# empymod/emg3d

Measured on AMD Instinct MI355X. Metric: Mcells/s per multigrid cycle, higher is better.
Workload: dtype c128

## Files before the change

emg3d_amd/csrc/emg3d_hip.hip:

```cpp
#include "../../include/emg3d_hip.h"

#include <cstring>
#include <new>

#include <chrono>
#include "mg.hpp"
#include "receivers.hpp"
#include "source.hpp"
#include "gradient.hpp"
#include "regrid.hpp"

#define EMG3D_HIP_VERSION EMG3D_HIP_ABI_VERSION

namespace {

template <class T>
MG<T>* as(emg3d_mg_t* mg) { return static_cast<MG<T>*>(reinterpret_cast<emg3d_mg*>(mg)); }

static int current_device() { int d = 0; if (hipGetDevice(&d) != hipSuccess) { (void)hipGetLastError(); d = 0; } return d; }

template <class T> static T scalar_of(double re, double im);
template <> double scalar_of<double>(double re, double) { return re; }
template <> c128 scalar_of<c128>(double re, double im) { return mk(re, im); }

// ... 460 lines not shown
    HIP_TRY(hipMemcpy(dv, values, (size_t)tot * sizeof(T), hipMemcpyHostToDevice));
    int rc = interp3d_device<T>(nullptr, dv, nn, 0, 1, nx, nx * ny, pts, n, xi, method, has_fill != 0, fill, cval, nullptr, scr, dout);
    if (rc == 0 && hipMemcpy(out, dout, (size_t)n * sizeof(T), hipMemcpyDeviceToHost) != hipSuccess) rc = (int)hipGetLastError();
        return rc;
}

}

template <class T>
static void* efield_ptr(MG<T>* m) {
    if (hipSetDevice(m->device) != hipSuccess) { (void)hipGetLastError(); return nullptr; }
    T* p = m->sel_e();
    m->check_launch();
    return m->err ? nullptr : (void*)p;
}

template <class T>
static int sweep_plan_impl(i64 nx, i64 ny, i64 nz, int dir, int order, int nsys, int cu_count, char* name, int64_t* info) {
    SweepKnobs K;
    if (cu_count > 0) K.simds = 4 * (i64)cu_count;
    else sweep_device_knobs<T>(K, current_device());
    K.order = order; K.nsys = nsys;
    const SweepPlan p = plan_sweep(K, SweepShape{{nx, ny, nz}, (int)sizeof(T)}, dir - 1);
    memcpy(name, p.name, sizeof p.name);
    info[0] = p.nmax; info[1] = p.lpw; info[2] = p.rounds; info[3] = p.fac_kind; info[4] = p.split ? 1 : 0; info[5] = p.big ? 1 : 0;
    return 0;
}

template <class T>
static int fuse_plan_impl(i64 nx, i64 ny, i64 nz, int dir, int order, int nsys, int cu_count, int npass, int own, int max_seg, i64 budget, int64_t* info,
                          int64_t* ranges, i64 nranges) {
    SweepKnobs K;
    if (cu_count > 0) K.simds = 4 * (i64)cu_count;
    else sweep_device_knobs<T>(K, current_device());
    K.order = order; K.nsys = nsys;
    if (own > 0) K.fuse_own = own;
    if (max_seg > 0) K.fuse_max_seg = max_seg;
    if (budget > 0) K.fuse_max_bytes = budget;
    const SweepShape G{{nx, ny, nz}, (int)sizeof(T)};
    const FusePlan f = plan_fuse(K, G, dir - 1, npass);
    int P, Q;
    sweep_axes(dir - 1, P, Q);
    info[0] = f.fused ? 1 : 0; info[1] = f.axis ? Q : P; info[2] = f.g.nX; info[3] = f.g.own; info[4] = f.g.nslabs; info[5] = f.g.npass;
    info[6] = f.nw; info[7] = f.scratch_bytes;
    if (!f.fused || !ranges) return 0;
    const i64 per = 4 + 2 * (i64)npass;
    if (nranges < per * f.g.nslabs) return -2;
    for (int k = 0; k < f.g.nslabs; ++k) {
        int64_t* r = ranges + per * k;
        r[0] = fuse_x0(f.g, k); r[1] = fuse_x1(f.g, k);
        i64 a = -1, b = -1;
        for (int j = 0; j <= f.g.nX; ++j) if (fuse_owner(f.g, j) == k) { if (a < 0) a = j; b = j + 1; }
        r[2] = a; r[3] = b;
        for (int p = 0; p < npass; ++p) { r[4 + 2 * p] = fuse_lo(f.g, k, p); r[5 + 2 * p] = fuse_hi(f.g, k, p); }
    }
    return 0;
}

template <class T>
static int jvec_stage(MG<T>* m, const double* const hv[3], const double* dv[3]) {
    Level<T>& L = *m->lv0;
    double* stage = reinterpret_cast<double*>(L.r);
    const i64 n = L.nCells;
    int used = 0;
    for (int c = 0; c < 3; ++c) {
        dv[c] = nullptr;
        if (!hv[c]) continue;
        for (int q = 0; q < c; ++q) if (hv[q] == hv[c]) dv[c] = dv[q];
        if (dv[c]) continue;
        double* d = stage + (i64)used++ * n;
        HIP_TRY(hipMemcpyAsync(d, hv[c], (size_t)n * sizeof(double), hipMemcpyHostToDevice, m->stream));
        dv[c] = d;
    }
    return 0;
}

template <class T>
static int jvec_source_impl(MG<T>* m, int efield_vec, double smu0_re, double smu0_im, const double* vx, const double* vy,
                            const double* vz) {
    if (sizeof(T) == 8 && smu0_im != 0.0) return -2;
    HIP_TRY(hipSetDevice(m->device));
    Level<T>& L = *m->lv0;
    const T* fwd = m->vec(efield_vec);
    if (!fwd || efield_vec < 0) return -2;
    const double* hv[3] = {vx, vy, vz};
    const double* dv[3];
    { const int st = jvec_stage<T>(m, hv, dv); if (st) return st; }
    T* s = m->sel_s();
    if (m->broken) return (int)hipErrorOutOfMemory;
    hipLaunchKernelGGL(k_jvec_source<T>, dim3((unsigned)((L.nE + 255) / 256)), dim3(256), 0, m->stream, L.nC[0], L.nC[1], L.nC[2],
                       L.fl, fwd, smu0_re, smu0_im, dv[0], dv[1], dv[2], (const double*)L.h[0], (const double*)L.h[1],
                       (const double*)L.h[2], s, L.nE);
    m->source_changed();
    m->lv0->s_dense = true;
    m->check_launch();
    return finish(m);
}

template <class T>
static int jvec_source_b_impl(MG<T>* m, int fwd_bvec, double smu0_re, double smu0_im, const double* vx, const double* vy,
                              const double* vz, const int32_t* use) {
    if (sizeof(T) == 8 && smu0_im != 0.0) return -2;
    HIP_TRY(hipSetDevice(m->device));
    Level<T>& L = *m->lv0;
    if (fwd_bvec < 0 || fwd_bvec >= (int)m->bvecs.size()) return -2;
    const T* fwd = m->bvecs[(size_t)fwd_bvec];
// ... 1146 lines not shown
```

emg3d_amd/csrc/mg.hpp:

```cpp
#pragma once
#include <algorithm>
#include <cmath>
#include <cstdlib>
#include <cstring>
#include <map>
#include <memory>
#include <mutex>
#include <chrono>
#include <vector>

#include "common.hpp"
#include "smooth.hpp"
#include "stencil.hpp"
#include "gradient.hpp"
#include "regrid.hpp"
#include "smooth_qpl.hpp"
#include "smooth_qc.hpp"
#include "smooth_thm.hpp"
#include "smooth_tha.hpp"
#include "sweep_launch.hpp"
#include "sweep_plan.hpp"

template <class T>
struct Level {
    i64 nC[3];
    i64 nE, nCells;
    FieldLayout fl;
    CellLayout cl;
    std::vector<double> h_host[3], nodes[3], centers[3];
    double* h[3] = {nullptr, nullptr, nullptr};
    double* ih[3] = {nullptr, nullptr, nullptr};
    T* eta[3] = {nullptr, nullptr, nullptr};
    double* zeta = nullptr;
    unsigned char* sflag[3] = {nullptr, nullptr, nullptr};
    bool sflag_valid[3] = {false, false, false};
    bool s_dense = false;
    bool zeta_sep = false;
    T *s = nullptr, *e = nullptr, *r = nullptr;
    T *eT = nullptr, *sT = nullptr;
    T* etaT[3] = {nullptr, nullptr, nullptr};
    double* zetaT = nullptr;
    bool sT_valid = false;
    FieldLayout flT;
    CellLayout clT;
    T *eW[2] = {nullptr, nullptr}, *sW[2] = {nullptr, nullptr};
    double* zetaW[2] = {nullptr, nullptr};
    bool sW_valid[2] = {false, false};
    int e_home = 0;
    T* fac[3] = {nullptr, nullptr, nullptr};
    void* qd[3][4] = {{nullptr, nullptr, nullptr, nullptr}, {nullptr, nullptr, nullptr, nullptr}, {nullptr, nullptr, nullptr, nullptr}};
    unsigned qdn[3][4] = {{0, 0, 0, 0}, {0, 0, 0, 0}, {0, 0, 0, 0}};
    T* fz[3] = {nullptr, nullptr, nullptr};
    i64 fz_n[3] = {0, 0, 0};
    FusePlan fuse[3];
    int fuse_key[3] = {-1, -1, -1};
    std::vector<int> passes[3];
    i64 fac_lines[3] = {0, 0, 0};
    i64 fac_mid[3] = {0, 0, 0};
    int fac_kind[3] = {0, 0, 0};
    SweepPlan plan[3];
    int plan_key[3] = {-1, -1, -1};
};

struct Transfer {
    int sc = -1;
    int co[3] = {0, 0, 0};
    double* w[3][3] = {{nullptr, nullptr, nullptr}, {nullptr, nullptr, nullptr}, {nullptr, nullptr, nullptr}};
    int* pidx[3] = {nullptr, nullptr, nullptr};
    double* pwt[3] = {nullptr, nullptr, nullptr};
};

template <class T>
struct Hierarchy {
    std::vector<std::shared_ptr<Level<T>>> lv;
    std::vector<Transfer> tr;
};

class DevicePool {
    std::mutex mu;
    struct Parked { void* p; int tag; };
    std::multimap<std::pair<int, size_t>, Parked> free_blocks;
    size_t held = 0, cap;
public:
    DevicePool() {
        const char* g = getenv("EMG3D_POOL_GB");
        cap = (size_t)((g ? atof(g) : 96.0) * (double)((size_t)1 << 30));
    }
    void* take(int device, size_t nb, int tag = 0, bool* hit = nullptr) {
        std::lock_guard<std::mutex> lk(mu);
        if (hit) *hit = false;
        auto rng = free_blocks.equal_range({device, nb});
        if (rng.first == rng.second) return nullptr;
        auto pick = rng.second;
        for (auto it = rng.first; it != rng.second; ++it) if (it->second.tag == tag) { pick = it; break; }
        if (pick == rng.second && tag != 0)
            for (auto it = rng.first; it != rng.second; ++it) if (it->second.tag == 0) { pick = it; break; }
        if (pick == rng.second) pick = rng.first;
        if (hit) *hit = tag != 0 && pick->second.tag == tag;
        void* p = pick->second.p;
        free_blocks.erase(pick);
        held -= nb;
        return p;
    }
    bool give(int device, void* p, size_t nb, int tag = 0) {
        std::lock_guard<std::mutex> lk(mu);
        if (held + nb > cap) return false;
// ... 1005 lines not shown
        L.e_home = 0;
    }
    void e_to_w1(Level<T>& L) {
        if (L.e_home == 1) return;
        ensure_work(L, 1);
        convert_field(L, L.eW[1], L.e, 1, true, true);
        L.e_home = 1;
    }

    int lex_loop = (int)LAB_ENV("EMG3D_LEX_LOOP", 1);
    void line_args(Level<T>& L, int dir, LineArgs<T>& a, bool sweep) {
        if (dir == 0) { a.L = 0; a.P = 1; a.Q = 2; }
        else if (dir == 1) { a.L = 1; a.P = 0; a.Q = 2; }
        else { a.L = 2; a.P = 0; a.Q = 1; }
        const SweepPlan& P = plan(L, dir);
        const bool sp = sweep && P.split;
        const bool t = (sp && dir == 0) ? true : P.xt;
        const int w = (dir == 0) ? 0 : 1;
        for (int q = 0; q < 3; ++q) {
            a.nC[q] = L.nC[q]; a.eta[q] = t ? L.etaT[q] : L.eta[q]; a.h[q] = L.h[q]; a.ih[q] = L.ih[q];
        }
        a.fl = t ? L.flT : L.fl; a.cl = t ? L.clT : L.cl;
        a.split = sp ? 1 : 0;
        if (sp) { a.e = L.eW[w]; a.s = L.sW[w]; a.zeta = L.zetaW[w]; }
        else { a.e = t ? L.eT : L.e; a.s = t ? L.sT : L.s; a.zeta = t ? L.zetaT : L.zeta; }
        const i64 nP = L.nC[a.P], nQ = L.nC[a.Q];
        a.nA[0] = (nP - 0) / 2; a.nA[1] = (nP - 1) / 2;
        const i64 nB[2] = {(nQ - 0) / 2, (nQ - 1) / 2};
        a.nB2[0] = nB[0]; a.nB2[1] = nB[1];
        i64 o = 0;
        for (int c = 0; c < 4; ++c) { a.base[c] = o; o += a.nA[c & 1] * nB[c >> 1]; }
        a.nLinesTot = o;
        a.fac = L.fac[dir];
        a.mid = L.fac[dir] ? L.fac_mid[dir] : L.nC[a.L] - 1;
        a.qm = (L.fac[dir] && L.fac_kind[dir] == 3) ? 2 : 0;
        a.fcomp = (L.fac[dir] && L.fac_kind[dir] == 4) ? 1 : 0;
        a.zsep = (sweep && L.zeta_sep && use_zsep) ? 1 : 0;
        a.sflag = (sweep && sflag_on(L, dir) && L.sflag[dir] && L.sflag_valid[dir]) ? L.sflag[dir] : nullptr;
        a.xcd = xcd_map;
        a.tile = q_tile;
        {
            const int ax[3] = {a.L, a.P, a.Q};
            a.rs.ihL = a.ih[a.L]; a.rs.ihP = a.ih[a.P]; a.rs.ihQ = a.ih[a.Q];
            a.rs.hL = a.h[a.L]; a.rs.hP = a.h[a.P]; a.rs.hQ = a.h[a.Q];
            a.rs.nL = (unsigned)a.nC[a.L]; a.rs.slot0 = 0;
            a.rs.nP = (unsigned)a.nC[a.P]; a.rs.nQ = (unsigned)a.nC[a.Q];
            a.rs.csL = (unsigned)a.cl.st[a.L]; a.rs.csP = (unsigned)a.cl.st[a.P]; a.rs.csQ = (unsigned)a.cl.st[a.Q];
            for (int c = 0; c < 3; ++c) {
                a.rs.off[c] = (unsigned)a.fl.off[ax[c]];
                for (int d = 0; d < 3; ++d) a.rs.st[c][d] = (unsigned)a.fl.st[ax[c]][ax[d]];
            }
        }
        a.qd = nullptr; a.qdn = 0;
        a.fe = nullptr; a.fnE = 0; a.fax = a.fnX = a.fown = a.fns = a.fnp = 0; a.fseq = 0;
        for (int c = 0; c < 4; ++c) { a.fqd[c] = nullptr; a.fqdn[c] = 0; }
        a.qpl = P.NW; a.qM = P.M; a.seg = P.seg; a.qlpw = 0;
        a.tha = P.helpers;
        a.mode = 0; a.cP = a.cQ = 0; a.cntA = a.cntB = 0; a.t = a.jQ0 = a.cnt = 0;
        a.bt = sweep ? batch(L) : Batch();
    }

    void ensure_factor(Level<T>& L, int dir) {
        const SweepPlan& P = plan(L, dir);
        if (P.xt) ensure_transposed_model(L);
        if (L.fac[dir]) return;
        L.fac_lines[dir] = (L.nC[dir == 0 ? 1 : 0] - 1) * (L.nC[dir == 2 ? 1 : 2] - 1);
        L.fac[dir] = dalloc<T>(L.fac_lines[dir] * P.fac_entries);
        L.fac_mid[dir] = P.mid;
        L.fac_kind[dir] = P.fac_kind;
        if (P.fac_kind == 3) thm_attrs();
        compute_factor(L, dir);
    }
    void compute_factor(Level<T>& L, int dir) {
        LineArgs<T> a;
        line_args(L, dir, a, false);
        a.fac = L.fac[dir];
        a.fcomp = L.fac_kind[dir] == 4;
        if (L.fac_kind[dir] == 3) {
            a.mid = L.fac_mid[dir];
            const i64 nQ_ = L.nC[a.Q];
            const i64 nmax_ = a.nA[0] * ((nQ_ - 0) / 2);
            a.mode = 3;
            if (nmax_ > 0)
                MG_LAUNCH(k_line_factor_m<T>, dim3((unsigned)((nmax_ + EMG_LINE_BLOCK - 1) / EMG_LINE_BLOCK), 4),
                                   dim3(EMG_LINE_BLOCK), 0, stream, a);
            check_launch();
            return;
        }
        a.mid = L.fac_mid[dir];
        const i64 nQ = L.nC[a.Q];
        const i64 nB[2] = {(nQ - 0) / 2, (nQ - 1) / 2};
        a.mode = 3; a.cP = a.cQ = 0; a.cntA = a.cntB = 0;
        const i64 nmax = a.nA[0] * nB[0];
#ifdef EMG3D_LAB
        if (LAB_ENV("EMG3D_FACTOR_PER_COLOUR", 0)) {
            for (int c = 0; c < 4; ++c) {
                a.mode = 0; a.cP = c & 1; a.cQ = c >> 1; a.cntA = a.nA[a.cP]; a.cntB = nB[a.cQ];
                const i64 n = a.cntA * a.cntB;
                if (n > 0)
                    MG_LAUNCH(k_line_factor<T>, dim3((unsigned)((n + EMG_LINE_BLOCK - 1) / EMG_LINE_BLOCK)),
                                       dim3(EMG_LINE_BLOCK), 0, stream, a);
            }
            check_launch();
            return;
        }
#endif
        if (nmax > 0)
// ... 207 lines not shown
            L.eW[w] = cands[best];
            block_tag[cands[best]] = 1 + w;
            for (int k = 0; k < R.tries; ++k) if (k != best) release(cands[k]);
            moved |= best != 0;
            if (getenv("EMG3D_LOG_SETUP")) {
                fprintf(stderr, "[place] working copy %d (%s-lines, %.0f MB): kept candidate %d of %d;", w, dir == 0 ? "x" : dir == 1 ? "y" : "z",
                        (double)n * sizeof(T) / 1048576.0, best, R.tries);
                for (int k = 0; k < R.tries; ++k) fprintf(stderr, " %.3f", R.ms[k]);
                fprintf(stderr, " ms per sweep\n");
            }
        }
        if (moved) drop_graphs();
        check_launch();
    }

    void colour_passes(Level<T>& L, int dir, int nu, std::vector<int>& seq) {
        int Pa, Qa;
        sweep_axes(dir, Pa, Qa);
        const i64 nP = L.nC[Pa], nQ = L.nC[Qa];
        int iback = 0, last_c = -1;
        seq.clear();
        for (int it = 0; it < nu; ++it) {
            iback = 1 - iback;
            for (int ch = 0; ch < 4; ++ch) {
                const int c = iback ? colour_perm_b[ch] : colour_perm[ch];
                if (skip_idempotent && c == last_c) continue;
                last_c = c;
                if (((nP - (c & 1)) / 2) * ((nQ - (c >> 1)) / 2) <= 0) continue;
                seq.push_back(c);
            }
        }
    }
    const FusePlan& ensure_fuse(Level<T>& L, int dir, int nu) {
        const int key = nu * 256 + order + 2 * nsys;
        if (L.fuse_key[dir] == key) return L.fuse[dir];
        FusePlan& F = L.fuse[dir];
        F = FusePlan();
        L.fuse_key[dir] = key;
        L.passes[dir].clear();
        if (order != 1) return F;
        colour_passes(L, dir, nu, L.passes[dir]);
        const std::vector<int>& seq = L.passes[dir];
        plan(L, dir);
        F = plan_fuse(knobs, SweepShape{{L.nC[0], L.nC[1], L.nC[2]}, (int)sizeof(T)}, dir, (int)seq.size());
        if (!F.fused) return F;
        for (int c : seq) if (!L.qd[dir][c]) { F.fused = false; return F; }
        const i64 need = (i64)nsys * F.g.nslabs * L.nE;
        if (L.fz_n[dir] < need) {
            T* z = try_alloc<T>(need);
            if (!z) { F.fused = false; return F; }
            if (L.fz[dir]) release(L.fz[dir]);
            L.fz[dir] = z; L.fz_n[dir] = need;
        }
        return F;
    }
    void smooth_fused(Level<T>& L, int dir, const SweepPlan& P, const FusePlan& F, const std::vector<int>& seq, const LineArgs<T>& a) {
        LineArgs<T> b = a;
        b.mode = 0; b.xcd = 0;
        b.fe = L.fz[dir]; b.fnE = L.nE; b.fax = F.axis;
        b.fnX = F.g.nX; b.fown = F.g.own; b.fns = F.g.nslabs; b.fnp = F.g.npass;
        b.fseq = 0;
        for (int p = 0; p < F.g.npass; ++p) b.fseq |= (unsigned long long)seq[(size_t)p] << (4 * p);
        for (int c = 0; c < 4; ++c) { b.fqd[c] = L.qd[dir][c]; b.fqdn[c] = L.qd[dir][c] ? L.qdn[dir][c] : 0u; }
        if (log_launches) fprintf(stderr, "[sweep] nC %lld %lld %lld L %d lines %lld kernel %s split %d fused passes %d slabs %d own %d\n", (long long)a.nC[0],
                                  (long long)a.nC[1], (long long)a.nC[2], a.L, (long long)a.nLinesTot, P.name, a.split, F.g.npass, F.g.nslabs, F.g.own);
        memcpy(sweep_name, P.name, sizeof sweep_name);
        if (broken) return;
        qpl_fused_launch<T>(P.family == SweepFamily::qpl_chain, bgrid((unsigned)F.g.nslabs), stream, b);
        ScatterArgs sa;
        sa.nE = L.nE; sa.g = F.g;
        int Pa, Qa;
        sweep_axes(dir, Pa, Qa);
        sa.ax = F.axis ? Qa : Pa;
        for (int c = 0; c < 3; ++c) {
            sa.off[c] = L.fl.off[c];
            sa.d0[c] = (unsigned)((c == 0) ? L.nC[0] : L.nC[0] + 1); sa.d1[c] = (unsigned)((c == 1) ? L.nC[1] : L.nC[1] + 1);
        }
        hipLaunchKernelGGL(k_scatter_slabs<T>, dim3((unsigned)((L.nE + EMG_BLOCK - 1) / EMG_BLOCK), (unsigned)nsys), dim3(EMG_BLOCK), 0, stream,
                           a.e, (const T*)L.fz[dir], sa, a.bt);
    }

    void smooth_line(Level<T>& L, int dir, int nu, bool conv_in = true, bool conv_out = true) {
        if (nu <= 0) return;
        ensure_factor(L, dir);
        ensure_qdesc(L, dir);
        const FusePlan& F = ensure_fuse(L, dir, nu);
        if (dry) { prepare_work(L, dir); return; }
        if (conv_in) to_work(L, dir);
        ensure_sflags(L, dir);
        LineArgs<T> a;
        line_args(L, dir, a, true);
        const SweepPlan& P = plan(L, dir);
        const i64 nP = L.nC[a.P], nQ = L.nC[a.Q];
        const i64 nB[2] = {(nQ - 0) / 2, (nQ - 1) / 2};
        if (order == 1) {
            if (F.fused) smooth_fused(L, dir, P, F, L.passes[dir], a);
            else for (int c : L.passes[dir]) {
                a.mode = 0; a.cP = c & 1; a.cQ = c >> 1;
                a.cntA = a.nA[a.cP]; a.cntB = nB[a.cQ];
                a.rs.slot0 = (unsigned)a.base[c];
                a.qd = L.qd[dir][c]; a.qdn = (L.qd[dir][c] ? L.qdn[dir][c] : 0u);
                launch_sweep(P, a, a.cntA * a.cntB);
            }
            nu = 0;
        }
        int iback = 0;
        for (int it = 0; it < nu; ++it) {
            iback = 1 - iback;
            {
                const i64 tmin = 3, tmax = (nP - 1) + 2 * (nQ - 1);
                if (lex_loop && a.qpl && a.qM == 1 && a.seg <= 16) {
                    LineArgs<T> b = a;
                    b.mode = 2; b.t = tmin; b.jQ0 = tmax; b.cnt = iback; b.xcd = 0;
                    const i64 maxn = std::min<i64>(nQ - 1, (nP - 1) / 2 + 1), quads = maxn * a.seg;
                    const int lnw = quads <= 16 ? 1 : quads <= 32 ? 2 : quads <= 64 ? 4 : 8;
                    if (!broken) qpl_launch<T>(lnw, 1, true, 0, false, bgrid(1), stream, b);
                    sweep_kernel_name(sweep_name, sizeof sweep_name, SweepFamily::qpl, (int)sizeof(T), lnw, 1);
                    continue;
                }
                for (i64 th = tmin; th <= tmax; ++th) {
                    const i64 tt = iback ? tmax - (th - tmin) : th;
// ... 290 lines not shown
```

emg3d_amd/csrc/smooth.hpp:

```cpp
#pragma once
#include "common.hpp"

#define EMG_LINE_BLOCK 64

template <class T>
struct LineArgs {
    int L, P, Q;
    i64 nC[3];
    FieldLayout fl;
    CellLayout cl;
    T* e;
    const T* s;
    const T* eta[3];
    const double* zeta;
    const double* h[3];
    const double* ih[3];
    int split;
    i64 mid;
    int xcd;
    int tile;
    struct Resolved {
        const double *ihL, *ihP, *ihQ;
        const double *hL, *hP, *hQ;
        unsigned nL, csL, csP, csQ;
        unsigned nP, nQ;
        unsigned slot0;
        unsigned off[3], st[3][3];
    } rs;
    Batch bt;
    int qm;
    int qpl;
    int qM, seg;
    const unsigned char* sflag;
    int zsep;
    int qlpw;
    int tha;
    int fcomp;
    T* fac;
    const void* qd;
    unsigned qdn;
    T* fe;
    i64 fnE;
    int fax, fnX, fown, fns, fnp;
    unsigned long long fseq;
    const void* fqd[4];
    unsigned fqdn[4];
    i64 nLinesTot;
    i64 base[4];
    i64 nA[2];
    i64 nB2[2];
    int mode;
    int cP, cQ;
    i64 cntA, cntB;
    i64 t, jQ0, cnt;
};

template <class T>
__device__ __forceinline__ bool line_of_thread(const LineArgs<T>& a, i64& jP, i64& jQ) {
    const i64 idx = (i64)blockIdx.x * blockDim.x + threadIdx.x;
    if (a.mode == 0) {
        if (idx >= a.cntA * a.cntB) return false;
        const i64 b = idx / a.cntA, q = idx - b * a.cntA;
        jP = 1 + a.cP + 2 * q;
        jQ = 1 + a.cQ + 2 * b;
    } else {
        if (idx >= a.cnt) return false;
        jQ = a.jQ0 + idx;
        jP = a.t - 2 * jQ;
    }
    return true;
}

template <class T>
__device__ __forceinline__ i64 line_slot(const LineArgs<T>& a, i64 jP, i64 jQ) {
    const int cP = (int)((jP - 1) & 1), cQ = (int)((jQ - 1) & 1);
    return a.base[cP + 2 * cQ] + ((jP - 1) >> 1) + a.nA[cP] * ((jQ - 1) >> 1);
}

struct LineCoef {
    double QP_Lm[2], PQ_Lm[2];
    double QL_Pm[2], LQ_Pm[2], QL_Pp[2], LQ_Pp[2];
    double PL_Qm[2], LP_Qm[2], PL_Qp[2], LP_Qp[2];
};

__device__ __forceinline__ void line_coef(LineCoef& c, const double z[2][2][2], const double kL[2],
                                          const double kP[2], const double kQ[2]) {
#pragma unroll
    for (int S = 0; S < 2; ++S) {
        c.QP_Lm[S] = kP[S] * (z[0][S][1] + z[0][S][0]);
        c.PQ_Lm[S] = kQ[S] * (z[0][1][S] + z[0][0][S]);
        c.QL_Pm[S] = kL[S] * (z[S][0][1] + z[S][0][0]);
        c.LQ_Pm[S] = kQ[S] * (z[1][0][S] + z[0][0][S]);
        c.QL_Pp[S] = kL[S] * (z[S][1][1] + z[S][1][0]);
        c.LQ_Pp[S] = kQ[S] * (z[1][1][S] + z[0][1][S]);
// ... 1136 lines not shown
```

emg3d_amd/csrc/smooth_qpl.hpp:

```cpp
#pragma once
#include "smooth.hpp"
#include "sweep_plan.hpp"


template <int K>
__device__ __forceinline__ double quad_bcast(double v) {
    constexpr int ctrl = K | (K << 2) | (K << 4) | (K << 6);
    int lo = __double2loint(v), hi = __double2hiint(v);
    lo = __builtin_amdgcn_update_dpp(0, lo, ctrl, 0xf, 0xf, false);
    hi = __builtin_amdgcn_update_dpp(0, hi, ctrl, 0xf, 0xf, false);
    return __hiloint2double(hi, lo);
}
template <int K>
__device__ __forceinline__ c128 quad_bcast(c128 v) { return mk(quad_bcast<K>(v.re), quad_bcast<K>(v.im)); }
__device__ __forceinline__ double quad_sum(double v) {
    int lo = __double2loint(v), hi = __double2hiint(v);
    double o = __hiloint2double(__builtin_amdgcn_update_dpp(0, hi, 0xb1, 0xf, 0xf, false),
                                __builtin_amdgcn_update_dpp(0, lo, 0xb1, 0xf, 0xf, false));
    v += o;
    lo = __double2loint(v); hi = __double2hiint(v);
    o = __hiloint2double(__builtin_amdgcn_update_dpp(0, hi, 0x4e, 0xf, 0xf, false),
                         __builtin_amdgcn_update_dpp(0, lo, 0x4e, 0xf, 0xf, false));
    return v + o;
}
__device__ __forceinline__ c128 quad_sum(c128 v) { return mk(quad_sum(v.re), quad_sum(v.im)); }

template <bool UP>
__device__ __forceinline__ double row_shift4(double v) {
    constexpr int ctrl = UP ? 0x114 : 0x104;
    int lo = __double2loint(v), hi = __double2hiint(v);
    lo = __builtin_amdgcn_update_dpp(0, lo, ctrl, 0xf, 0xf, false);
    hi = __builtin_amdgcn_update_dpp(0, hi, ctrl, 0xf, 0xf, false);
    return __hiloint2double(hi, lo);
}
template <bool UP> __device__ __forceinline__ c128 row_shift4(c128 v) { return mk(row_shift4<UP>(v.re), row_shift4<UP>(v.im)); }
template <bool UP> __device__ __forceinline__ double lane_shift4(double v) { return UP ? __shfl_up(v, 4) : __shfl_down(v, 4); }
template <bool UP> __device__ __forceinline__ c128 lane_shift4(c128 v) { return mk(lane_shift4<UP>(v.re), lane_shift4<UP>(v.im)); }

template <class T>
__device__ __forceinline__ void qpl_args_burst(const LineArgs<T>& a) {
    asm volatile("" :: "s"(a.e), "s"(a.s), "s"(a.fac), "s"(a.zeta), "s"(a.rs.ihL), "s"(a.rs.ihP), "s"(a.rs.ihQ), "s"(a.bt.st),
                 "s"(a.bt.mask), "s"(a.bt.n), "s"(a.xcd), "s"(a.mode), "s"(a.cntA), "s"(a.cntB), "s"(a.cP), "s"(a.cQ), "s"(a.seg),
                 "s"(a.rs.nL), "s"(a.rs.csL), "s"(a.rs.csP), "s"(a.rs.csQ), "s"(a.rs.slot0), "s"(a.rs.off[0]), "s"(a.rs.off[1]),
                 "s"(a.rs.off[2]));
    asm volatile("" :: "s"(a.rs.st[0][0]), "s"(a.rs.st[0][1]), "s"(a.rs.st[0][2]), "s"(a.rs.st[1][0]), "s"(a.rs.st[1][1]),
                 "s"(a.rs.st[1][2]), "s"(a.rs.st[2][0]), "s"(a.rs.st[2][1]), "s"(a.rs.st[2][2]), "s"(a.t), "s"(a.jQ0), "s"(a.cnt),
                 "s"(a.rs.nP), "s"(a.rs.nQ), "s"(a.qd), "s"(a.qdn));
}

template <class T, int NW, int M, bool HL = false, int DM = 0, bool CH = false, bool FZ = false>
__global__ __launch_bounds__(64 * NW) void k_line_sweep_qpl(LineArgs<T> a) {
    static_assert(DM == 0 || (!HL && (NW == 1 || FZ)), "descriptors: one wave per workgroup, colour order");
    static_assert(!CH || ((NW == 1 || FZ) && M == 1 && !HL), "chain form: lines inside one wave, one block per quad");
    static_assert(!FZ || (DM == 2 && M == 1 && !HL), "fused passes: descriptors, one block per quad, colour order");
    constexpr int NQ = 16 * NW;
#ifdef EMG3D_LAB
    long long qts[7] = {0, 0, 0, 0, 0, 0, 0};
#define QPL_TS(i) do { if (a.tile & 512) { asm volatile("" ::: "memory"); qts[i] = (long long)__builtin_readcyclecounter(); asm volatile("" ::: "memory"); } } while (0)
#else
#define QPL_TS(i) do {} while (0)
#endif
    QPL_TS(0);
    qpl_args_burst(a);
    QPL_TS(1);
    const int tid = threadIdx.x;
    const int quad = tid >> 2, r = tid & 3;
    const int seg = a.seg;
    const int ch = quad & (seg - 1);
    const int lseg = __builtin_ctz((unsigned)seg);
    const int lpg = NQ >> lseg;
    typedef unsigned int u32;
    EMG_SWEEP_WG(a)
    __shared__ T xb[2][(FZ && CH) ? 1 : NQ][4][5];
    T* const ebase = FZ ? a.fe + ((i64)bsys_ * a.fns + wg) * a.fnE : a.e + boff_;
    const void* qd_ = a.qd;
    u32 qdn_ = a.qdn;
    u32 tix = (u32)wg * (64u * NW) + (u32)tid;
    auto one = [&](const u32 gline, const u32 nlines, const u32 t_, const u32 jQ0_) {
    const bool live = gline < nlines;
    const int nL = (int)a.rs.nL;
    auto ld_d = [](const double* base, u32 idx) -> double { return *reinterpret_cast<const double*>(reinterpret_cast<const char*>(base) + idx * 8u); };
    auto ld_t = [](const T* base, u32 idx) -> T { return *reinterpret_cast<const T*>(reinterpret_cast<const char*>(base) + idx * (u32)sizeof(T)); };
    const T* __restrict__ e = ebase;
    const T* __restrict__ s = (a.s + boff_);
    T Wr[M][5], W0[M][5];
    T b[M][5];
    double av[M][4], dv[M][4];
    bool lastb[M], inl[M];
    u32 dS[M], dS0[M];
    constexpr int QD_U4 = 3, QD_D2 = 8;
    if constexpr (DM == 2) {
        const uint4* const q4 = reinterpret_cast<const uint4*>(qd_);
        const emg_d2* const c2 = reinterpret_cast<const emg_d2*>(q4 + (size_t)(QD_U4 * M) * qdn_);
        uint4 u[M][QD_U4];
        emg_d2 cf[M][QD_D2];
#pragma unroll
        for (int j = 0; j < M; ++j) {
#pragma unroll
            for (int k = 0; k < QD_U4; ++k) u[j][k] = q4[(u32)(QD_U4 * j + k) * qdn_ + tix];
#pragma unroll
// ... 336 lines not shown
            cmac(t0, mG[0], quad_bcast<0>(dn)); cmac(t1, mG[3], quad_bcast<3>(dn)); cmac(t0, mG[2], quad_bcast<2>(dn));
            vc = inner ? t0 + t1 : mc;
        }
        const T dn = from_above(vc);
        v[0] = quad_bcast<0>(dn); v[1] = quad_bcast<1>(dn); v[2] = quad_bcast<2>(dn); v[3] = quad_bcast<3>(dn);
        if (!inner) { v[0] = Zero<T>::v(); v[1] = Zero<T>::v(); v[2] = Zero<T>::v(); v[3] = Zero<T>::v(); }
    } else {
#pragma unroll
    for (int j = M - 2; j >= 0; --j) {
        publish(p);
        sync();
        bwd_row(j);
        compose_with(p, quad);
        p ^= 1;
    }
#pragma unroll 1
    for (int st = 1; st < seg; st <<= 1) {
        publish(p);
        sync();
        if (ch + st < seg) { if (2 * st < seg) compose_with(p, quad + st); else compose_c_only(p, quad + st); }
        p ^= 1;
    }
    publish(p);
    sync();
#pragma unroll
    for (int k = 0; k < 4; ++k) v[k] = (ch + 1 < seg) ? xb[p][quad + 1][k][0] : Zero<T>::v();
    }
    QPL_TS(5);
    T* eo = ebase;
#pragma unroll
    for (int j = M - 1; j >= 0; --j) {
        T x0 = z0[j], xr = zr[j];
#pragma unroll
        for (int l = 0; l < 4; ++l) { cmsc(x0, W0[j][l + 1], v[l]); cmsc(xr, Wr[j][l + 1], v[l]); }
        const int i = ch * M + j;
        if (live && inl[j]) {
            if (r == 0) eo[dS0[j]] = x0;
            if (!lastb[j]) eo[dS[j]] = xr;
        }
        if (j > 0) {
            const double ar = (r == 0) ? av[j][0] : (r == 1) ? av[j][1] : (r == 2) ? av[j][2] : av[j][3];
            const double dr = (r == 0) ? dv[j][0] : (r == 1) ? dv[j][1] : (r == 2) ? dv[j][2] : dv[j][3];
            T vr = x0 * ar;
            cmac(vr, xr, dr);
            v[0] = quad_bcast<0>(vr); v[1] = quad_bcast<1>(vr); v[2] = quad_bcast<2>(vr); v[3] = quad_bcast<3>(vr);
        }
    }
    QPL_TS(6);
    };

    if constexpr (FZ) {
        const FuseGeom g{a.fnX, a.fown, a.fns, a.fnp};
        const int k = (int)wg;
        {
            T* __restrict__ dst = ebase;
            const T* __restrict__ src = a.e + boff_;
            const int ra = fuse_lo(g, k, 0) - 1, rb = fuse_hi(g, k, 0) + 1;
            const int X = a.fax ? 2 : 1;
            const u32 nO = a.fax ? a.rs.nP : a.rs.nQ;
#pragma unroll
            for (int c = 0; c < 3; ++c) {
                const u32 dL = a.rs.nL + (c != 0 ? 1u : 0u), dX = (u32)g.nX + (c != X ? 1u : 0u), dO = nO + ((c == 0 || c == X) ? 1u : 0u);
                const int rbc = rb < (int)dX - 1 ? rb : (int)dX - 1;
                if (rbc < ra) continue;
                const u32 w = (u32)(rbc - ra + 1);
                const u32 stL = a.rs.st[c][0], stX = a.fax ? a.rs.st[c][2] : a.rs.st[c][1], stO = a.fax ? a.rs.st[c][1] : a.rs.st[c][2];
                const bool xf = stX < stL;
                const u32 n0 = xf ? w : dL, n1 = xf ? dL : w, tot = n0 * n1 * dO;
                for (u32 idx = (u32)tid; idx < tot; idx += 64u * NW) {
                    const u32 t = idx / n0, i0 = idx - t * n0, i2 = t / n1, i1 = t - i2 * n1;
                    const u32 iX = (u32)ra + (xf ? i0 : i1), iL = xf ? i1 : i0;
                    const u32 off = a.rs.off[c] + iL * stL + iX * stX + i2 * stO;
                    dst[off] = src[off];
                }
            }
        }
        __threadfence_block();
        __syncthreads();
        const u32 lslot = (u32)(quad >> lseg), wslot0 = (u32)(((tid >> 6) * 16) >> lseg);
        for (int p = 0; p < g.npass; ++p) {
            const int c = (int)((a.fseq >> (4 * p)) & 3ull);
            const int cP = c & 1, cQ = c >> 1;
            const u32 cA = (u32)a.nA[cP], cB = (u32)a.nB2[cQ];
            const int cX = a.fax ? cQ : cP;
            const u32 qa = (u32)(fuse_lo(g, k, p) - cX) >> 1, qb = (u32)(fuse_hi(g, k, p) + 1 - cX) >> 1;
            const u32 nx = qb > qa ? qb - qa : 0u;
            const u32 nloc = nx * (a.fax ? cA : cB);
            qd_ = a.fqd[c]; qdn_ = a.fqdn[c];
            for (u32 base = 0; base < nloc; base += (u32)lpg) {
                if (base + wslot0 < nloc) {
                    const u32 m = base + lslot;
                    const bool lv = m < nloc;
                    const u32 mm = lv ? m : base + wslot0;
                    u32 qq, bq;
                    if (a.fax == 0) { bq = mm / nx; qq = qa + (mm - bq * nx); }
                    else { const u32 t = mm / cA; qq = mm - t * cA; bq = qa + t; }
                    const u32 gl = bq * cA + qq;
                    tix = ((gl >> (4 - lseg)) << 6) + ((((gl & ((16u >> lseg) - 1u)) << lseg) + (u32)ch) << 2) + (u32)r;
                    one(lv ? 0u : 1u, 1u, 0u, 0u);
                }
            }
            __threadfence_block();
            __syncthreads();
        }
    } else if constexpr (!HL) {
        one((u32)wg * (u32)lpg + (u32)(quad >> lseg), (u32)((a.mode == 0) ? a.cntA * a.cntB : a.cnt), (u32)a.t, (u32)a.jQ0);
#ifdef EMG3D_LAB
        if ((a.tile & 512) && blockIdx.x == 0 && threadIdx.x == 0) {
            asm volatile("s_waitcnt vmcnt(0)" ::: "memory");
            const long long tend = (long long)__builtin_readcyclecounter();
            printf("[qpl<%d,%d> seg %d lines %lld] args %lld loads issued %lld loads in + coefficients %lld forward %lld backward %lld stores issued %lld stores done %lld (cycles after entry)\n",
                   NW, M, seg, (long long)(a.cntA * a.cntB), qts[1] - qts[0], qts[2] - qts[0], qts[3] - qts[0], qts[4] - qts[0], qts[5] - qts[0], qts[6] - qts[0], tend - qts[0]);
        }
#endif
    } else {
        const int nPm = (int)a.rs.nP - 1, nQm = (int)a.rs.nQ - 1;
        const int tmin = (int)a.t, tmax = (int)a.jQ0;
        for (int th = tmin; th <= tmax; ++th) {
            const int tt = a.cnt ? tmax - (th - tmin) : th;
            const int lo = tt - nPm;
            int jq0 = lo <= 0 ? 1 : (lo + 1) / 2;
            if (jq0 < 1) jq0 = 1;
            int jq1 = (tt - 1) / 2;
            if (jq1 > nQm) jq1 = nQm;
            const int n = jq1 - jq0 + 1;
            for (int base = 0; base < n; base += lpg) {
                one((u32)(quad >> lseg), (u32)min(n - base, lpg), (u32)tt, (u32)(jq0 + base));
                __threadfence_block();
                __syncthreads();
            }
        }
    }
#undef QPL_TS
}
```

emg3d_amd/csrc/sweep_plan.hpp:

```cpp
#pragma once
#include <algorithm>
#include <cstdint>
#include <cstdio>
#include <cstdlib>

typedef int64_t i64;

#ifndef LAB_ENV
#ifdef EMG3D_LAB
inline long long lab_env_(const char* name, long long def) { const char* v = getenv(name); return v ? atoll(v) : def; }
inline int lab_env_ch_(const char* name) { const char* v = getenv(name); return v ? v[0] : 0; }
#define LAB_ENV(name, def) lab_env_(name, (long long)(def))
#define LAB_ENV_CH(name) lab_env_ch_(name)
#else
#define LAB_ENV(name, def) ((long long)(def))
#define LAB_ENV_CH(name) 0
#endif
#endif

constexpr int SWEEP_THA_LPW = 8, SWEEP_THA_RING = 8, SWEEP_THA_MAX_DYN_LDS = 140 * 1024, SWEEP_THA_STATIC_LDS = 18 * 1024;
inline i64 sweep_tha_lds_bytes(i64 nL, int tsize) {
    return (2 * SWEEP_THA_RING * 5 + 2 * ((nL + 1) / 2 + 2)) * (5 * SWEEP_THA_LPW) * (i64)tsize;
}

struct SweepKnobs {
    i64 simds = 1024;
    i64 lds_limit = 160 * 1024;
    bool tha_lds_granted = true;
    int order = 1, nsys = 1;
    int batch_tune = getenv("EMG3D_BATCH_TUNE") ? atoi(getenv("EMG3D_BATCH_TUNE")) : 0;

    int sweep_kernel = LAB_ENV_CH("EMG3D_SWEEP") == 't' ? 1 : 0;
    bool use_xt = LAB_ENV("EMG3D_XT", 1) != 0;
    i64 xt_min_cells = LAB_ENV("EMG3D_XT_MIN", 8192);
    int th_lpw = (int)LAB_ENV("EMG3D_TH_LPW", 0);
    int force_lpw = (int)LAB_ENV("EMG3D_LPW", 0);
    bool use_twist = LAB_ENV("EMG3D_TWIST", 1) != 0;
    i64 twist_max_lines_env = LAB_ENV("EMG3D_TWIST_MAX", 0);
    int tw_stages = (int)LAB_ENV("EMG3D_TW_STAGES", 0);
    int use_split = (int)LAB_ENV("EMG3D_SPLIT", 2);
    i64 split_min_cells = LAB_ENV("EMG3D_SPLIT_MIN_CELLS", 2000000);
    int use_q = (int)LAB_ENV("EMG3D_Q", 1);
    i64 q_min_lines_env = LAB_ENV("EMG3D_Q_MIN_LINES", 0);
    int q_stages = (int)LAB_ENV("EMG3D_Q_STAGES", 0);
    int q_lpw = (int)LAB_ENV("EMG3D_Q_LPW", 0);
    int q_big_lab = (int)LAB_ENV("EMG3D_Q_BIG", 0);
    int use_qpl = (int)LAB_ENV("EMG3D_QPL", 7);
    i64 qpl_min_nl = LAB_ENV("EMG3D_QPL_MIN", 2);
    i64 qpl_max_nl = LAB_ENV("EMG3D_QPL_MAX_NL", 64);
    i64 qpl_m2_min = LAB_ENV("EMG3D_QPL_M2", 32);
    int qpl_chain_seg = (int)LAB_ENV("EMG3D_QPL_CHAIN", 4);
    i64 qpl_few_lines_env = LAB_ENV("EMG3D_QPL_FEW", 0);
    i64 qpl_max_lines = LAB_ENV("EMG3D_QPL_MAX", (i64)1 << 40);
    int use_qdesc = (int)LAB_ENV("EMG3D_QDESC", 1);
    i64 qdesc_max_threads_env = LAB_ENV("EMG3D_QDESC_MAX", 0);
    int fuse_max_seg = (int)LAB_ENV("EMG3D_QPL_FUSE", 4);
    i64 fuse_own = LAB_ENV("EMG3D_QPL_FUSE_W", 0);
    i64 fuse_max_bytes = LAB_ENV("EMG3D_QPL_FUSE_BYTES", (i64)64 << 20);
    int use_tha = (int)LAB_ENV("EMG3D_THA", 3);
    i64 tha_min_nl = LAB_ENV("EMG3D_THA_MIN", 33), tha_mid_nl = LAB_ENV("EMG3D_THA_MID", 64), tha_min_lines_env = LAB_ENV("EMG3D_THA_MIN_LINES", 0);
    i64 tha_max_nl = LAB_ENV("EMG3D_THA_MAX", 128);
    i64 tha_big_max_lines_env = LAB_ENV("EMG3D_THA_BIG_LINES", 0);
    int tha_split = (int)LAB_ENV("EMG3D_THA_SPLIT", 0);

    i64 q_min_lines() const { return q_min_lines_env > 0 ? q_min_lines_env : 8 * simds; }
    i64 twist_max_lines() const { return twist_max_lines_env > 0 ? twist_max_lines_env : q_min_lines(); }
    i64 qpl_few_lines() const { return qpl_few_lines_env > 0 ? qpl_few_lines_env : simds; }
    i64 qdesc_max_threads() const { return qdesc_max_threads_env > 0 ? qdesc_max_threads_env : (9000 * simds + 1023) / 1024; }
    i64 tha_min_lines() const { return tha_min_lines_env > 0 ? tha_min_lines_env : (1100 * simds + 1023) / 1024; }
    i64 tha_big_max_lines() const { return tha_big_max_lines_env > 0 ? tha_big_max_lines_env : (i64)SWEEP_THA_LPW * (simds / 4); }
};

struct SweepShape {
    i64 nC[3];
    int tsize;
    i64 cells() const { return nC[0] * nC[1] * nC[2]; }
    i64 edges() const {
        return nC[0] * (nC[1] + 1) * (nC[2] + 1) + (nC[0] + 1) * nC[1] * (nC[2] + 1) + (nC[0] + 1) * (nC[1] + 1) * nC[2];
    }
    i64 lines(int dir) const { return (nC[dir == 0 ? 1 : 0] / 2) * (nC[dir == 2 ? 1 : 2] / 2); }
    i64 lines_tot(int dir) const { return (nC[dir == 0 ? 1 : 0] - 1) * (nC[dir == 2 ? 1 : 2] - 1); }
    i64 field_stride(int c, int ax, bool transposed) const {
        const i64 d0 = (c == 0) ? nC[0] : nC[0] + 1, d1 = (c == 1) ? nC[1] : nC[1] + 1;
        return ax == 2 ? d0 * d1 : ((ax == 0) != transposed) ? 1 : (transposed ? d1 : d0);
    }
    i64 cell_stride(int ax, bool transposed) const {
        return ax == 2 ? nC[0] * nC[1] : ((ax == 0) != transposed) ? 1 : (transposed ? nC[1] : nC[0]);
    }
};

enum class SweepFamily { tpl, rp, qc, qc_big, thm, tha, qpl, qpl_chain };

inline void sweep_kernel_name(char* out, size_t len, SweepFamily f, int tsize, int p1 = 0, int p2 = 0) {
    static const char* const base[] = {"k_line_sweep", "k_line_sweep_rp", "k_line_sweep_qc", "k_line_sweep_qc_big", "k_line_sweep_thm",
                                       "k_line_sweep_tha", "k_line_sweep_qpl", "k_line_sweep_qpl_chain"};
    const char* tn = tsize == 16 ? "c128" : "f64";
    if (f == SweepFamily::tpl) snprintf(out, len, "%s<%s>", base[(int)f], tn);
    else if (f == SweepFamily::rp || f == SweepFamily::tha) snprintf(out, len, "%s<%s,%d>", base[(int)f], tn, p1);
    else snprintf(out, len, "%s<%s,%d,%d>", base[(int)f], tn, p1, p2);
}

struct SweepPlan {
    SweepFamily family = SweepFamily::tpl;
    int stages = 0, inst_lpw = 0, helpers = 0, NW = 0, M = 0, seg = 0;
    int qlpw = 0;
    bool big = false;
    bool split = false;
    bool xt = false;
    int work_id = 0;
    int fac_kind = 0;
    i64 fac_entries = 0;
// ... 85 lines not shown
        p1 = p.helpers;
        p.lpw = SWEEP_THA_LPW; p.rounds = (((nmax + p.lpw - 1) / p.lpw) * K.nsys + S / 4 - 1) / (S / 4);
    } else if (p.fac_kind == 3) {
        p.family = SweepFamily::thm;
        const i64 lines = nmax * K.nsys, r8 = (2 * ((lines + 7) / 8) + S - 1) / S, r12 = (2 * ((lines + 11) / 12) + S - 1) / S;
        p.inst_lpw = (K.th_lpw == 4 || K.th_lpw == 8 || K.th_lpw == 12) ? K.th_lpw : (23 * r12 < 20 * r8) ? 12 : 8;
        p.stages = K.tw_stages ? K.tw_stages : 3;
        p1 = p.stages; p2 = p.inst_lpw;
        p.lpw = p.inst_lpw; p.rounds = (2 * ((nmax + p.lpw - 1) / p.lpw) * K.nsys + S - 1) / S;
    } else if (qpl) {
        p.M = (nL >= K.qpl_m2_min) ? 2 : 1;
        p.seg = 4; while (p.seg < (nL + p.M - 1) / p.M) p.seg *= 2;
        p.NW = p.seg <= 16 ? 1 : p.seg / 16;
        p.family = (p.NW == 1 && p.M == 1 && K.order == 1 && p.seg <= K.qpl_chain_seg) ? SweepFamily::qpl_chain : SweepFamily::qpl;
        p1 = p.NW; p2 = p.M;
        p.fac_entries = 15 * (i64)p.M * p.seg;
        p.lpw = (16 * p.NW) / p.seg; p.rounds = (((nmax + p.lpw - 1) / p.lpw) * p.NW * K.nsys + S - 1) / S;
        p.qdesc = K.use_qdesc && K.order == 1 && p.NW == 1 && G.lines_tot(dir) * p.fac_entries < ((i64)1 << 32) &&
                  ((nmax + p.lpw - 1) / p.lpw) * 64 <= K.qdesc_max_threads();
    } else if ((rp_fits || p.big) && p.fac_kind == 4) {
        p.family = p.big ? SweepFamily::qc_big : SweepFamily::qc;
        p.inst_lpw = p.big ? 16 : K.q_lpw ? K.q_lpw : (nmax >= K.q_min_lines() ? 16 : 4);
        p.stages = (K.q_stages == 2 || K.q_stages == 3) ? K.q_stages
                 : (p.inst_lpw == 16 && nmax * K.nsys > 15 * S && nmax * K.nsys <= 16 * S) ? 2 : 3;
        p.qlpw = p.inst_lpw == 16 ? sweep_balanced_lpw(K, nmax * K.nsys) : p.inst_lpw;
        p1 = p.stages; p2 = p.inst_lpw;
        p.lpw = p.qlpw; p.rounds = (((nmax + p.lpw - 1) / p.lpw) * K.nsys + S - 1) / S;
    } else if (rp_fits || p.big) {
        p.family = SweepFamily::rp;
        p.lpw = K.force_lpw ? K.force_lpw : (nmax >= 8 * S ? 8 : 4);
        p.inst_lpw = (p.lpw == 8 || p.lpw == 12) ? (int)p.lpw : 4;
        p1 = p.inst_lpw;
        p.rounds = (((nmax + p.lpw - 1) / p.lpw) * K.nsys + S - 1) / S;
    } else {
        p.family = SweepFamily::tpl;
        p.lpw = 64; p.rounds = (((nmax + 63) / 64) * K.nsys + S - 1) / S;
    }
    sweep_kernel_name(p.name, sizeof p.name, p.family, G.tsize, p1, p2);
    return p;
}

constexpr int SWEEP_FUSE_MAX_PASSES = 16;
#if defined(__HIPCC__)
#define SWEEP_HD __host__ __device__
#else
#define SWEEP_HD
#endif
struct FuseGeom { int nX, own, nslabs, npass; };
SWEEP_HD inline int fuse_x0(const FuseGeom& g, int k) { return 1 + k * g.own; }
SWEEP_HD inline int fuse_x1(const FuseGeom& g, int k) { const int x = 1 + (k + 1) * g.own; return (k == g.nslabs - 1 || x > g.nX) ? g.nX : x; }
SWEEP_HD inline int fuse_lo(const FuseGeom& g, int k, int p) { const int v = fuse_x0(g, k) - (g.npass - 1 - p); return v < 1 ? 1 : v; }
SWEEP_HD inline int fuse_hi(const FuseGeom& g, int k, int p) { const int v = fuse_x1(g, k) + (g.npass - 1 - p); return v > g.nX - 1 ? g.nX - 1 : v; }
SWEEP_HD inline int fuse_owner(const FuseGeom& g, int j) { const int k = j <= 0 ? 0 : (j - 1) / g.own; return k > g.nslabs - 1 ? g.nslabs - 1 : k; }

struct FusePlan {
    bool fused = false;
    int axis = 0;
    int nw = 0;
    FuseGeom g = {0, 0, 0, 0};
    i64 scratch_bytes = 0;
};
inline void sweep_axes(int dir, int& P, int& Q) { P = dir == 0 ? 1 : 0; Q = dir == 2 ? 1 : 2; }
inline FusePlan plan_fuse(const SweepKnobs& K, const SweepShape& G, int dir, int npass) {
    FusePlan f;
    const SweepPlan p = plan_sweep(K, G, dir);
    if (K.order != 1 || (p.family != SweepFamily::qpl && p.family != SweepFamily::qpl_chain) || p.NW != 1 || p.M != 1 || !p.qdesc) return f;
    if (p.seg > K.fuse_max_seg || p.seg > 8 || npass < 3 || npass > SWEEP_FUSE_MAX_PASSES) return f;
#ifndef EMG3D_LAB
    if (p.family != SweepFamily::qpl_chain) return f;
#endif
    int P, Q;
    sweep_axes(dir, P, Q);
    f.axis = G.nC[Q] > G.nC[P] ? 1 : 0;
    const i64 nX = G.nC[f.axis ? Q : P];
    if (nX < 2 || nX > (1 << 20)) return f;
    i64 own = K.fuse_own > 0 ? K.fuse_own : 2;
    own = std::min<i64>(own, nX - 1);
    f.g.nX = (int)nX; f.g.own = (int)own; f.g.nslabs = (int)((nX - 1 + own - 1) / own); f.g.npass = npass;
    f.nw = p.family == SweepFamily::qpl_chain ? 8 : 4;
    f.scratch_bytes = (i64)K.nsys * f.g.nslabs * G.edges() * (i64)G.tsize;
    f.fused = f.scratch_bytes <= K.fuse_max_bytes;
    return f;
}
```

Baseline: 254.0.

## Write fused-sweep results back from owner slabs into a double buffer, skipping scatter

New measurement: 255.3, median of 6. No clear change (+0.5%).

```diff
diff --git a/emg3d_amd/csrc/emg3d_hip.hip b/emg3d_amd/csrc/emg3d_hip.hip
--- a/emg3d_amd/csrc/emg3d_hip.hip
+++ b/emg3d_amd/csrc/emg3d_hip.hip
@@ -536,6 +536,7 @@
         i64 a = -1, b = -1;
         for (int j = 0; j <= f.g.nX; ++j) if (fuse_owner(f.g, j) == k) { if (a < 0) a = j; b = j + 1; }
         r[2] = a; r[3] = b;
+        if (a != fuse_wb_lo(f.g, k) || b != fuse_wb_hi(f.g, k) + 1) return -7;
         for (int p = 0; p < npass; ++p) { r[4 + 2 * p] = fuse_lo(f.g, k, p); r[5 + 2 * p] = fuse_hi(f.g, k, p); }
     }
     return 0;
diff --git a/emg3d_amd/csrc/mg.hpp b/emg3d_amd/csrc/mg.hpp
--- a/emg3d_amd/csrc/mg.hpp
+++ b/emg3d_amd/csrc/mg.hpp
@@ -52,6 +52,7 @@
     unsigned qdn[3][4] = {{0, 0, 0, 0}, {0, 0, 0, 0}, {0, 0, 0, 0}};
     T* fz[3] = {nullptr, nullptr, nullptr};
     i64 fz_n[3] = {0, 0, 0};
+    T* e2 = nullptr;
     FusePlan fuse[3];
     int fuse_key[3] = {-1, -1, -1};
     std::vector<int> passes[3];
@@ -1163,7 +1164,7 @@
             }
         }
         a.qd = nullptr; a.qdn = 0;
-        a.fe = nullptr; a.fnE = 0; a.fax = a.fnX = a.fown = a.fns = a.fnp = 0; a.fseq = 0;
+        a.fe = nullptr; a.fo = nullptr; a.fnE = 0; a.fax = a.fnX = a.fown = a.fns = a.fnp = 0; a.fseq = 0;
         for (int c = 0; c < 4; ++c) { a.fqd[c] = nullptr; a.fqdn[c] = 0; }
         a.qpl = P.NW; a.qM = P.M; a.seg = P.seg; a.qlpw = 0;
         a.tha = P.helpers;
@@ -1477,21 +1478,29 @@
             if (L.fz[dir]) release(L.fz[dir]);
             L.fz[dir] = z; L.fz_n[dir] = need;
         }
+        if (!L.e2 && plan_fuse_writeback(knobs, F, &L == lv0.get())) L.e2 = try_alloc<T>(L.nE);
         return F;
     }
     void smooth_fused(Level<T>& L, int dir, const SweepPlan& P, const FusePlan& F, const std::vector<int>& seq, const LineArgs<T>& a) {
         LineArgs<T> b = a;
         b.mode = 0; b.xcd = 0;
+        const bool wb = plan_fuse_writeback(knobs, F, &L == lv0.get()) && L.e2 && a.e == L.e;
+        b.fo = wb ? L.e2 : nullptr;
         b.fe = L.fz[dir]; b.fnE = L.nE; b.fax = F.axis;
         b.fnX = F.g.nX; b.fown = F.g.own; b.fns = F.g.nslabs; b.fnp = F.g.npass;
         b.fseq = 0;
         for (int p = 0; p < F.g.npass; ++p) b.fseq |= (unsigned long long)seq[(size_t)p] << (4 * p);
         for (int c = 0; c < 4; ++c) { b.fqd[c] = L.qd[dir][c]; b.fqdn[c] = L.qd[dir][c] ? L.qdn[dir][c] : 0u; }
-        if (log_launches) fprintf(stderr, "[sweep] nC %lld %lld %lld L %d lines %lld kernel %s split %d fused passes %d slabs %d own %d\n", (long long)a.nC[0],
-                                  (long long)a.nC[1], (long long)a.nC[2], a.L, (long long)a.nLinesTot, P.name, a.split, F.g.npass, F.g.nslabs, F.g.own);
+        if (log_launches) fprintf(stderr, "[sweep] nC %lld %lld %lld L %d lines %lld kernel %s split %d fused passes %d slabs %d own %d %s\n", (long long)a.nC[0],
+                                  (long long)a.nC[1], (long long)a.nC[2], a.L, (long long)a.nLinesTot, P.name, a.split, F.g.npass, F.g.nslabs, F.g.own,
+                                  wb ? "owner write-back" : "scatter launch");
         memcpy(sweep_name, P.name, sizeof sweep_name);
         if (broken) return;
         qpl_fused_launch<T>(P.family == SweepFamily::qpl_chain, bgrid((unsigned)F.g.nslabs), stream, b);
+        if (wb) {
+            std::swap(L.e, L.e2);
+            return;
+        }
         ScatterArgs sa;
         sa.nE = L.nE; sa.g = F.g;
         int Pa, Qa;
diff --git a/emg3d_amd/csrc/smooth.hpp b/emg3d_amd/csrc/smooth.hpp
--- a/emg3d_amd/csrc/smooth.hpp
+++ b/emg3d_amd/csrc/smooth.hpp
@@ -40,6 +40,7 @@
     const void* qd;
     unsigned qdn;
     T* fe;
+    T* fo;
     i64 fnE;
     int fax, fnX, fown, fns, fnp;
     unsigned long long fseq;
diff --git a/emg3d_amd/csrc/smooth_qpl.hpp b/emg3d_amd/csrc/smooth_qpl.hpp
--- a/emg3d_amd/csrc/smooth_qpl.hpp
+++ b/emg3d_amd/csrc/smooth_qpl.hpp
@@ -45,7 +45,7 @@
                  "s"(a.rs.off[2]));
     asm volatile("" :: "s"(a.rs.st[0][0]), "s"(a.rs.st[0][1]), "s"(a.rs.st[0][2]), "s"(a.rs.st[1][0]), "s"(a.rs.st[1][1]),
                  "s"(a.rs.st[1][2]), "s"(a.rs.st[2][0]), "s"(a.rs.st[2][1]), "s"(a.rs.st[2][2]), "s"(a.t), "s"(a.jQ0), "s"(a.cnt),
-                 "s"(a.rs.nP), "s"(a.rs.nQ), "s"(a.qd), "s"(a.qdn));
+                 "s"(a.rs.nP), "s"(a.rs.nQ), "s"(a.qd), "s"(a.qdn), "s"(a.fo));
 }
 
 template <class T, int NW, int M, bool HL = false, int DM = 0, bool CH = false, bool FZ = false>
@@ -488,10 +488,7 @@
     if constexpr (FZ) {
         const FuseGeom g{a.fnX, a.fown, a.fns, a.fnp};
         const int k = (int)wg;
-        {
-            T* __restrict__ dst = ebase;
-            const T* __restrict__ src = a.e + boff_;
-            const int ra = fuse_lo(g, k, 0) - 1, rb = fuse_hi(g, k, 0) + 1;
+        auto copy_range = [&](T* __restrict__ dst, const T* __restrict__ src, const int ra, const int rb) {
             const int X = a.fax ? 2 : 1;
             const u32 nO = a.fax ? a.rs.nP : a.rs.nQ;
 #pragma unroll
@@ -510,7 +507,8 @@
                     dst[off] = src[off];
                 }
             }
-        }
+        };
+        copy_range(ebase, a.e + boff_, fuse_lo(g, k, 0) - 1, fuse_hi(g, k, 0) + 1);
         __threadfence_block();
         __syncthreads();
         const u32 lslot = (u32)(quad >> lseg), wslot0 = (u32)(((tid >> 6) * 16) >> lseg);
@@ -539,6 +537,7 @@
             __threadfence_block();
             __syncthreads();
         }
+        if (a.fo) copy_range(a.fo + boff_, ebase, fuse_wb_lo(g, k), fuse_wb_hi(g, k));
     } else if constexpr (!HL) {
         one((u32)wg * (u32)lpg + (u32)(quad >> lseg), (u32)((a.mode == 0) ? a.cntA * a.cntB : a.cnt), (u32)a.t, (u32)a.jQ0);
 #ifdef EMG3D_LAB
diff --git a/emg3d_amd/csrc/sweep_plan.hpp b/emg3d_amd/csrc/sweep_plan.hpp
--- a/emg3d_amd/csrc/sweep_plan.hpp
+++ b/emg3d_amd/csrc/sweep_plan.hpp
@@ -57,6 +57,7 @@
     int fuse_max_seg = (int)LAB_ENV("EMG3D_QPL_FUSE", 4);
     i64 fuse_own = LAB_ENV("EMG3D_QPL_FUSE_W", 0);
     i64 fuse_max_bytes = LAB_ENV("EMG3D_QPL_FUSE_BYTES", (i64)64 << 20);
+    int tail = (int)LAB_ENV("EMG3D_TAIL", 1);
     int use_tha = (int)LAB_ENV("EMG3D_THA", 3);
     i64 tha_min_nl = LAB_ENV("EMG3D_THA_MIN", 33), tha_mid_nl = LAB_ENV("EMG3D_THA_MID", 64), tha_min_lines_env = LAB_ENV("EMG3D_THA_MIN_LINES", 0);
     i64 tha_max_nl = LAB_ENV("EMG3D_THA_MAX", 128);
@@ -248,6 +249,8 @@
 SWEEP_HD inline int fuse_lo(const FuseGeom& g, int k, int p) { const int v = fuse_x0(g, k) - (g.npass - 1 - p); return v < 1 ? 1 : v; }
 SWEEP_HD inline int fuse_hi(const FuseGeom& g, int k, int p) { const int v = fuse_x1(g, k) + (g.npass - 1 - p); return v > g.nX - 1 ? g.nX - 1 : v; }
 SWEEP_HD inline int fuse_owner(const FuseGeom& g, int j) { const int k = j <= 0 ? 0 : (j - 1) / g.own; return k > g.nslabs - 1 ? g.nslabs - 1 : k; }
+SWEEP_HD inline int fuse_wb_lo(const FuseGeom& g, int k) { return k == 0 ? 0 : fuse_x0(g, k); }
+SWEEP_HD inline int fuse_wb_hi(const FuseGeom& g, int k) { return k == g.nslabs - 1 ? g.nX : (k + 1) * g.own; }
 
 struct FusePlan {
     bool fused = false;
@@ -278,3 +281,6 @@
     f.fused = f.scratch_bytes <= K.fuse_max_bytes;
     return f;
 }
+inline bool plan_fuse_writeback(const SweepKnobs& K, const FusePlan& f, bool level0) {
+    return f.fused && K.tail >= 1 && !level0 && K.nsys == 1;
+}
```
